# Evrytania/LTE-Cell-Scanner

Measured on AMD Instinct MI355X. Metric: capture-buffers/s (1.92 Msps, 153600-samp) full CellSearch; HBM GB/s vs peak, higher is better.
Workload: dtype i8 x 3 base-256 digits of 24-bit integer templates, i32 accumulate (exact)

## Files before the change

__graft_entry__.py:

```python
from __future__ import annotations

import importlib.util
import os
import subprocess
import sys

ROOT = os.path.dirname(os.path.abspath(__file__))
PKG_DIR = os.path.join(ROOT, "lte-cell-scanner_amd")
CSRC = os.path.join(PKG_DIR, "csrc")
LIB = os.path.join(PKG_DIR, "liblcs_amd.so")
HIP_SOURCES = ["pss_xcorr.hip", "pss_xcorr_i8.hip", "pss_xcorr_f16.hip", "peak_search.hip", "sss_foe.hip", "tfg_mib.hip", "cell_meas.hip", "tfg_wide.hip", "pcfich.hip", "pdcch.hip", "pdsch.hip", "tracker.hip", "channelizer.hip", "channelizer_rate.hip", "lcs_api.hip", "lte_tables.cpp"]
HIPCC_FLAGS = ["--offload-arch=gfx950", "-O3", "-std=c++17", "-ffp-contract=off", "-fPIC", "-shared",
               "-Wall", "-Wno-unused-function"]


_CHAN_DEPS = [os.path.join(CSRC, "channelizer.h"), os.path.join(CSRC, "lcs_internal.h"), os.path.join(ROOT, "include", "lcs.h")]
HOST_TWINS = [
    ("vit_host.cpp", "libvit_host.so", [os.path.join(CSRC, "lte_device.h")], []),
    ("cut_host.cpp", "libcut_host.so", [os.path.join(CSRC, "lte_device.h")], []),
    ("probe_host.cpp", "libprobe_host.so", [os.path.join(CSRC, "lte_device.h")], ["-pthread"]),
    ("pss_ref_host.cpp", "libpss_ref_host.so", [os.path.join(CSRC, "pss_ref.h"), os.path.join(CSRC, "lcs_internal.h"), os.path.join(CSRC, "xcorr_route.h")], []),
    ("chan_rate_host.cpp", "libchan_rate_host.so", _CHAN_DEPS, []),
    ("chan_u8_host.cpp", "libchan_u8_host.so", _CHAN_DEPS, []),
    ("chan_args_host.cpp", "libchan_args_host.so", _CHAN_DEPS, []),
    ("chan_stream_host.cpp", "libchan_stream_host.so", _CHAN_DEPS, []),
    ("chan_stream_u8_host.cpp", "libchan_stream_u8_host.so", _CHAN_DEPS, []),
    ("screen_bound_host.cpp", "libscreen_bound_host.so", [os.path.join(CSRC, "screen_bound.h")], []),
    ("xc_route_host.cpp", "libxc_route_host.so", [os.path.join(CSRC, "xcorr_route.h")], []),
    ("foe_coarse_host.cpp", "libfoe_coarse_host.so", [os.path.join(CSRC, "foe_coarse.h"), os.path.join(CSRC, "lte_device.h")], []),
    ("tdd_config_host.cpp", "libtdd_config_host.so", [os.path.join(CSRC, "tdd_config.h"), os.path.join(CSRC, "lte_device.h")], []),
    ("cell_meas_host.cpp", "libcell_meas_host.so", [os.path.join(CSRC, "cell_meas.h"), os.path.join(CSRC, "tdd_config.h"), os.path.join(CSRC, "lte_device.h")], []),
    ("meas_wide_host.cpp", "libmeas_wide_host.so", [os.path.join(CSRC, "cell_meas_wide.h"), os.path.join(CSRC, "cell_meas.h"), os.path.join(CSRC, "tdd_config.h"), os.path.join(CSRC, "lte_device.h")], []),
    ("pcfich_host.cpp", "libpcfich_host.so", [os.path.join(CSRC, "pcfich.h"), os.path.join(CSRC, "cell_meas.h"), os.path.join(CSRC, "tdd_config.h"), os.path.join(CSRC, "lte_device.h"), os.path.join(ROOT, "include", "lcs.h")], []),
    ("pdcch_host.cpp", "libpdcch_host.so", [os.path.join(CSRC, "pdcch.h"), os.path.join(CSRC, "pcfich.h"), os.path.join(CSRC, "cell_meas.h"), os.path.join(CSRC, "tdd_config.h"), os.path.join(CSRC, "lte_device.h"), os.path.join(ROOT, "include", "lcs.h")], []),
    ("pdsch_host.cpp", "libpdsch_host.so", [os.path.join(CSRC, "pdsch.h"), os.path.join(CSRC, "pdcch.h"), os.path.join(CSRC, "pcfich.h"), os.path.join(CSRC, "cell_meas.h"), os.path.join(CSRC, "tdd_config.h"), os.path.join(CSRC, "lte_device.h"), os.path.join(ROOT, "include", "lcs.h")], []),
    ("pdsch_comb_host.cpp", "libpdsch_comb_host.so", [os.path.join(ROOT, "tests", "host", "pdsch_host.cpp"), os.path.join(CSRC, "pdsch_comb.h"), os.path.join(CSRC, "pdsch.h"), os.path.join(CSRC, "pdcch.h"), os.path.join(CSRC, "pcfich.h"), os.path.join(CSRC, "cell_meas.h"), os.path.join(CSRC, "tdd_config.h"), os.path.join(CSRC, "lte_device.h"), os.path.join(ROOT, "include", "lcs.h")], []),
    ("pdsch_dvrb_host.cpp", "libpdsch_dvrb_host.so", [os.path.join(ROOT, "tests", "host", "pdsch_host.cpp"), os.path.join(CSRC, "pdsch.h"), os.path.join(CSRC, "pdcch.h"), os.path.join(CSRC, "pcfich.h"), os.path.join(CSRC, "cell_meas.h"), os.path.join(CSRC, "tdd_config.h"), os.path.join(CSRC, "lte_device.h"), os.path.join(ROOT, "include", "lcs.h")], []),
    ("pbch_host.cpp", "libpbch_host.so", [os.path.join(CSRC, "lte_tables.cpp"), os.path.join(CSRC, "lcs_internal.h")], []),
    ("trk_layout_host.cpp", "libtrk_layout_host.so", [os.path.join(CSRC, "trk_layout.h"), os.path.join(ROOT, "include", "lcs.h")], []),
]


def load_package():
    name = "lte_cell_scanner_amd"
    if name in sys.modules:
        return sys.modules[name]
    path = os.path.join(PKG_DIR, "__init__.py")
    spec = importlib.util.spec_from_file_location(name, path, submodule_search_locations=[PKG_DIR])
    mod = importlib.util.module_from_spec(spec)
    sys.modules[name] = mod
    spec.loader.exec_module(mod)
    return mod


def _newer(target, sources):
    if not os.path.exists(target):
        return True
    t = os.path.getmtime(target)
    return any(os.path.getmtime(s) > t for s in sources)


def build(force: bool = False) -> None:
    hipcc = os.environ.get("HIPCC", "/opt/rocm/bin/hipcc")
    srcs = [os.path.join(CSRC, s) for s in HIP_SOURCES if os.path.exists(os.path.join(CSRC, s))]
    deps = srcs + [os.path.join(CSRC, "lcs_internal.h"), os.path.join(CSRC, "lcs_mem.h"), os.path.join(CSRC, "channelizer.h"), os.path.join(CSRC, "lte_device.h"), os.path.join(CSRC, "foe_coarse.h"), os.path.join(CSRC, "tdd_config.h"), os.path.join(CSRC, "cell_meas.h"), os.path.join(CSRC, "cell_meas_wide.h"), os.path.join(CSRC, "pcfich.h"), os.path.join(CSRC, "pdcch.h"), os.path.join(CSRC, "pdsch.h"), os.path.join(CSRC, "pdsch_comb.h"), os.path.join(CSRC, "tfg_layout.h"), os.path.join(CSRC, "trk_layout.h"), os.path.join(CSRC, "pss_ref.h"), os.path.join(CSRC, "xcorr_route.h"), os.path.join(CSRC, "screen_bound.h"), os.path.join(ROOT, "include", "lcs.h")]
    if force or _newer(LIB, deps):
        subprocess.check_call([hipcc] + HIPCC_FLAGS + ["-o", LIB] + srcs)
    mk = os.path.join(ROOT, "host", "Makefile")
    if os.path.exists(mk):
        subprocess.check_call(["make", "-C", os.path.dirname(mk), "-s"] + (["-B"] if force else []))
    subprocess.check_call(["make", "-C", os.path.join(ROOT, "oracle"), "-s"])
    for src, lib, extra_deps, extra_flags in HOST_TWINS:
        src, lib = os.path.join(ROOT, "tests", "host", src), os.path.join(ROOT, "tests", "host", lib)
        if os.path.exists(src) and (force or _newer(lib, [src] + extra_deps)):
            subprocess.check_call([hipcc, "--offload-arch=gfx950", "-O2", "-std=c++17", "-ffp-contract=off", "-fPIC", "-shared"] + extra_flags +
                                  ["-I" + os.path.join(ROOT, "include"), "-o", lib, src])
    pkg = load_package()
    pkg.capi.load()


def smoke() -> None:
    import numpy as np
    sys.path.insert(0, os.path.join(ROOT, "oracle"))
    import oracle as O
    pkg = load_package()
    g = np.load(os.path.join(ROOT, "tests", "golden", "capbuf_0000.npz"))
    iq = g["iq_u8"].astype(np.float64)
    cap = ((iq[0::2] - 127.0) / 128.0) + 1j * ((iq[1::2] - 127.0) / 128.0)
    fc = float(g["fc"][0])
    f = np.array([30e3, 35e3, 40e3])
    with pkg.Searcher(0) as s:
        r = s.xcorr_pss(cap, f, 2, fc, fc, 1.92e6, want_incoherent=False)
        Z = pkg.z_th1(r["sp_incoherent"], r["n_comb_xc"])
        peaks = s.peak_search(r["pow"], r["frq"], Z, f, fc, fc, r["single"], 2)
        r32 = s.xcorr_pss(0.5 * cap, f, 2, fc, fc, 1.92e6, want_incoherent=False)
        assert s.last_xcorr_info()[0].startswith("k_xcorr_mfma_blk"), s.last_xcorr_info()
    O.set_threads(min(8, os.cpu_count() or 1))
    ro = O.xcorr_pss(cap, f, 2, fc, fc, 1.92e6)
    assert np.array_equal(r32["frq"], ro["frq"]), "fp32 kernel: collapsed frequency indices differ from the oracle"
    assert np.allclose(4.0 * r32["pow"], ro["pow"], rtol=1e-5, atol=0)
    rel = np.abs(r["single"] - ro["single"]).max() / ro["single"].max()
    assert np.array_equal(r["frq"], ro["frq"]), "int8 kernel: collapsed frequency indices differ from the oracle"
    assert np.allclose(r["pow"], ro["pow"], rtol=1e-5, atol=0), "collapsed powers differ from the oracle"
    po = O.peak_search(ro["pow"], ro["frq"], O.z_th1(ro["sp_incoherent"], ro["n_comb_xc"]), f, fc, fc, ro["single"], 2)
    assert [(p.n_id_2, p.ind, p.freq) for p in peaks] == [(p.n_id_2, p.ind, p.freq) for p in po]
    import torch
    d = torch.from_numpy(np.ascontiguousarray(g["iq_u8"])).to("cuda:0")
    with pkg.Searcher(0) as s:
        cells = s.search_batch(d.data_ptr(), pkg.FMT_IQ_U8, 1, cap.size, f, fc, fc, 1.92e6, pkg.STAGE_FULL)[0]
    co, _ = O.search_capbuf(cap, f, fc, fc, 1.92e6)
# ... 20 lines not shown
```

lte-cell-scanner_amd/csrc/lcs_internal.h:

```cpp
#pragma once
#include <hip/hip_runtime.h>
#include <stdint.h>
#include <cstddef>
#include <string>
#include <type_traits>
#include <vector>
#include "../../include/lcs.h"
#include "lcs_mem.h"
#include "trk_layout.h"
#include "xcorr_route.h"

#define FS_LTE 30720000.0
#define LCS_NW_MAX 16
#define LCS_NF_LIMIT 1024
#define LCS_TAIL_PRIO() __builtin_amdgcn_s_setprio(3)
#define LCS_TG 16
#define LCS_LAG_TILE 64
#define LCS_PS 336
#define LCS_MAXP LCS_MAX_PEAKS
#define LCS_FRQ_TIE_EPS 4e-6f
#define LCS_I8_KB 5
#define LCS_I8_IMG 17024
#define LCS_I8_LAGS 512
#define LCS_I8_TILES ((LCS_N_IDX + LCS_I8_LAGS - 1) / LCS_I8_LAGS)
// ... 97 lines not shown
  int peak;
};

enum class FrqRepair {
  all,
  peaks_only,
  none_keep_2nd
};
struct Launch {
  int n_buf = 0;
  uint32_t n_cap = 0;
  XcGeom geo{};
  const SlotParams *params = nullptr;
  const double *fset = nullptr;
  XcKernel xc = XcKernel::fp32;
  CapSrc src{};
  FrqRepair repair = FrqRepair::all;
  bool screen = false;
  bool single_stream = false;
  bool needed_rows_only = false;
  int grid_items = 64;
  int round_cells = 0;
  int tfoec_parts = 4;
  const int16_t *tracked = nullptr;
  const int *n_tracked = nullptr;
  int duplex = LCS_DUPLEX_FDD;
  int foe_unwrap = 0;
  int tdd_config = 0;
  int cell_meas = 0;
};
struct BatchRecord {
  Launch l;
  int stage_mask = 0;
  int fmt = 0;
  int cell_rounds = 0;
  bool list_ops_counted = false;
};

struct StreamHost {
  SlotParams p;
  int n_tracked;
  int pad_;
  int16_t tracked[504];
  double f;
  lcs_cell res[LCS_MAXP];
  int n_peaks;
  int n_work[4];
};

#define LCS_STREAM_IN_BYTES (offsetof(StreamHost, f) + sizeof(double))

struct TrkStreamCell {
  std::vector<double> fo, ft, late;
  double bpo_before_tail = 0;
  long long tail_start = 0;
  long long n_seen = 0;
  long long next_raw[4] = {1, 1, 1, 1};
  long long ce_upto[4] = {0, 0, 0, 0};
  long long mib_next = 0;
  int cp_type = 0, n_id_1 = -1, n_id_2 = -1, n_ports = 0;
};
struct TrkStream {
  std::vector<TrkStreamCell> cells;
  DevBuf<double2> d_tail[3], d_spare[3];
};
struct TrkCutCap { size_t n_cells = 0, n = 0; };
template <int FIRST, int N, class Cap> struct TrkPart {
  DevBuf<char> buf[N];
  Cap cap;
  template <class T> T *at(const TrkLay &l, int a) const { return l.at<T>(buf[TRK_ROWS[a].buf - FIRST].get(), a); }
  int regrow(lcs_ctx *c, const TrkLay &l, const Cap &want);
  int reserve(lcs_ctx *c, TrkShape s) { return trk_fits(cap, s) ? LCS_OK : regrow(c, trk_layout(trk_grow(cap, s)), trk_grow(cap, s)); }
};

struct I8Set {
  DevBuf<uint16_t> cap8;
  DevBuf<uint16_t> cap8s;
  DevBuf<uint32_t> brow8;
  DevBuf<double> tq;
  DevBuf<float> tsc;
  DevBuf<int> scr_state;
  DevBuf<int> scr_tile;
  DevBuf<unsigned> scr_items;
  DevBuf<float> scr_zmin;
  bool ready = false;
};
struct F16Set {
  DevBuf<uint32_t> cap16h, cap16l;
  DevBuf<uint32_t> brow16;
  DevBuf<int> texp16;
  DevBuf<float> tsc16;
  DevBuf<unsigned> xmax16;
  DevBuf<unsigned> xpart16;
  bool ready = false;
};
struct XcBufs {
  I8Set i8;
  F16Set f16;
  DevBuf<float> btab;
};

struct lcs_ctx;
template <class Rec> struct SideTable {
  explicit SideTable(int sentinel_word) : sentinel(sentinel_word) {}
  DevBuf<Rec> tab;
  bool made = false;
  const int sentinel;
  Rec *get() const { return tab.get(); }
  int begin(lcs_ctx *c, int n_buf, bool on);
  int read_last(lcs_ctx *c, int n_buf, const Rec &none, int32_t Rec::*key, Rec *out, int max_cells_per_buf);
};

struct lcs_ctx_queues {
  int device = 0;
  hipStream_t stream = nullptr;
  hipStream_t stream_xc = nullptr;
  hipEvent_t ev_pre = nullptr, ev_post = nullptr;
  hipEvent_t ev_xc0 = nullptr, ev_xc1 = nullptr;
  hipEvent_t ev_stage[2] = {nullptr, nullptr};
  hipEvent_t ev_chan_slot[2] = {nullptr, nullptr};
  hipEvent_t ev_chan0 = nullptr, ev_chan1 = nullptr;
  ~lcs_ctx_queues();
};

struct lcs_ctx : lcs_ctx_queues {
  ~lcs_ctx();
  std::string err;

  int cap_slots = 0;
  uint32_t cap_n_cap = 0;
  int cap_n_f = 0;
  int cap_G = 0;
  bool cap_debug = false;

  DevBuf<float2> cap32;
  XcBufs xcb;
  DevBuf<double2> cap64;
  DevBuf<SlotParams> params_ws;
  DevBuf<double> fset_ws;
  DevBuf<float2> tmpl;
  DevBuf<int> start, smin, kp2;
  DevBuf<float> single, incoh, sref;
  DevBuf<double> pow_, work, spinc, zth, sp;
  DevBuf<int> frq;
  DevBuf<unsigned> fix_list;
  DevBuf<int> n_fix;
  DevBuf<float> second32;
  DevBuf<double> fset_g;
  DevBuf<lcs_cell> peaks;
  DevBuf<int> npeaks;
  DevBuf<float2> xc;
  DevBuf<WorkItem> pk_items;
  DevBuf<int> n_pk;
  DevBuf<double> sss_ws;
  DevBuf<WorkItem> work_items;
  DevBuf<int> n_work;
  DevBuf<double2> tfg;
  DevBuf<double2> tfg_comp;
  DevBuf<double2> ce;
  DevBuf<char> tfg_desc;
  DevBuf<double> tfg_ts;
  DevBuf<double> tfg_ts_comp;
  DevBuf<double> cell_scratch;
  DevBuf<lcs_cell> cells_out;
  DevBuf<double2> d_pss_td;
  DevBuf<double2> d_pss_fd;
  DevBuf<int8_t> d_sss_fd;
// ... 267 lines not shown
```

lte-cell-scanner_amd/csrc/pss_xcorr.hip:

```cpp
#include "lcs_internal.h"
#include "lte_device.h"
#include "pss_ref.h"
#include <algorithm>

typedef float f32x4 __attribute__((ext_vector_type(4)));

#define NW LCS_NW_MAX
#define NFM geo.n_f
#define GM geo.G

__global__ void k_ingest(const void *__restrict__ src, int fmt, uint32_t n_cap, float2 *__restrict__ cap32,
                         const double2 *__restrict__ cap64) {
  LCS_TAIL_PRIO();
  const int slot = blockIdx.y;
  const size_t base = (size_t)slot * n_cap;
  for (uint32_t i = blockIdx.x * blockDim.x + threadIdx.x; i < n_cap; i += gridDim.x * blockDim.x) {
    if (fmt == LCS_FMT_C64) {
      cap32[base + i] = ((const float2 *)src)[base + i];
    } else {
      const double2 v = cap64[base + i];
      cap32[base + i] = make_float2((float)v.x, (float)v.y);
    }
  }
}
// ... 333 lines not shown
  const int slot = blockIdx.y, i0 = blockIdx.x * SPI_TILE, tid = threadIdx.x, lane = tid & 63, wv = tid >> 6;
  const uint16_t *cap = cap8 + (size_t)slot * lcs_cap8_stride(n_cap);
  double acc[4] = {0, 0, 0, 0};
  for (int m = 0; m < a.n_comb_sp; ++m) {
    const uint32_t base = (uint32_t)m * 9600u + i0;
    int v[SPI_PER], run = 0;
#pragma unroll
    for (int j = 0; j < SPI_PER; ++j) {
      const int k = tid * SPI_PER + j;
      int pw = 0;
      if (k < SPI_N && base + k < n_cap) {
        const uint32_t s = cap[base + k];
        const int re = (int)(int8_t)(s & 255u), im = (int)(int8_t)(s >> 8);
        pw = re * re + im * im;
      }
      run += pw;
      v[j] = run;
    }
    int incl = run;
#pragma unroll
    for (int off = 1; off < 64; off <<= 1) { const int up = __shfl_up(incl, off); if (lane >= off) incl += up; }
    __syncthreads();
    if (lane == 63) wsum[wv] = incl;
    __syncthreads();
    int before = incl - run;
    for (int q = 0; q < wv; ++q) before += wsum[q];
    if (tid == 0) C[0] = 0;
#pragma unroll
    for (int j = 0; j < SPI_PER; ++j) { const int k = tid * SPI_PER + j; if (k < SPI_N) C[k + 1] = before + v[j]; }
    __syncthreads();
#pragma unroll
    for (int r = 0; r < 4; ++r) {
      const int i = tid + 256 * r;
      if (i < SPI_TILE) acc[r] += ((double)(C[i + 274] - C[i]) / 16384.0) / 274;
    }
  }
#pragma unroll
  for (int r = 0; r < 4; ++r) {
    const int i = i0 + tid + 256 * r;
    if (tid + 256 * r < SPI_TILE && i < 9600) {
      const double vv = acc[r] / a.n_comb_sp;
      const int o = (i + 137) % 9600;
      spinc[(size_t)slot * 9600 + o] = vv;
      zth[(size_t)slot * 9600 + o] = lcs_z_th1(a, vv);
    }
  }
}

struct CollapseBest { float v; int foi; float s; };
__device__ __forceinline__ void collapse_step(CollapseBest &b, float xe, int foi) {
  const bool tk = xe > b.v;
  b.s = __builtin_amdgcn_fmed3f(xe, b.v, b.s);
  b.v = tk ? xe : b.v;
  b.foi = tk ? foi : b.foi;
}
__device__ __forceinline__ void collapse_merge(CollapseBest &b, int lane_xor) {
  const float ov = __shfl_xor(b.v, lane_xor);
  const float os = __shfl_xor(b.s, lane_xor);
  const int of = __shfl_xor(b.foi, lane_xor);
  const bool tk = ov > b.v || (ov == b.v && of < b.foi);
  b.s = fmaxf(fminf(b.v, ov), fmaxf(b.s, os));
  b.v = tk ? ov : b.v;
  b.foi = tk ? of : b.foi;
}
__device__ __forceinline__ void collapse_flag(const CollapseBest &r, unsigned pos, unsigned *__restrict__ fix_list, int *__restrict__ n_fix,
                                              const double *__restrict__ zth) {
  if (!fix_list) return;
  if (r.v > 0.f && r.s >= r.v * (1.0f - LCS_FRQ_TIE_EPS)) {
    if (zth && (double)r.v < 0.999 * zth[(pos / (3 * LCS_N_IDX)) * LCS_N_IDX + pos % LCS_N_IDX]) return;
    fix_list[atomicAdd(n_fix, 1)] = pos;
  }
}
typedef const __attribute__((address_space(1))) char *collapse_gptr;
typedef float collapse_f4 __attribute__((ext_vector_type(4)));
__device__ __forceinline__ float4 collapse_row(collapse_gptr base, unsigned byte_off) {
  const collapse_f4 r = *reinterpret_cast<const __attribute__((address_space(1))) collapse_f4 *>(base + byte_off);
  return make_float4(r.x, r.y, r.z, r.w);
}
template <int DS, bool INCOH, bool LIST = false>
__global__ __launch_bounds__(256) void k_collapse(const float *__restrict__ sg, float *__restrict__ incoh,
                                                   double *__restrict__ pow_, float *__restrict__ pow32,
                                                   int *__restrict__ frq, unsigned *__restrict__ fix_list, int *__restrict__ n_fix,
                                                   const double *__restrict__ zth, float *__restrict__ second32, XcGeom geo, int n_buf,
                                                   const int *__restrict__ tile_flag = nullptr, const float *__restrict__ zmin = nullptr) {
  LCS_TAIL_PRIO();
  constexpr int CT = 64;
  static_assert(LCS_N_IDX % CT == 0 && LCS_TG == 16, "k_collapse tiles 9600 positions x 16 columns");
  constexpr int NT = LCS_N_IDX / CT;
  constexpr int NA = DS > 0 ? DS : 1;
  const int tid = threadIdx.x, q = tid & 3;
  const int ds = (DS >= 0) ? DS : min(geo.ds, 8);
  const float dsn = (float)(2 * geo.ds + 1);
  for (int vb = blockIdx.x; vb < NT * n_buf; vb += gridDim.x) {
    const int slot = vb / NT;
    const int idx = (vb % NT) * CT + (tid >> 2);
    bool mine = true;
    if (LIST) {
      static_assert(LCS_I8_LAGS % CT == 0, "a workgroup's positions lie in one lag tile");
      const int *tf = tile_flag + slot * LCS_I8_TILES;
      const int t0 = (vb % NT) * CT / LCS_I8_LAGS;
      if (!tf[t0]) continue;
      const int lo = idx - ds < 0 ? idx - ds + LCS_N_IDX : idx - ds, hi = idx + ds >= LCS_N_IDX ? idx + ds - LCS_N_IDX : idx + ds;
      mine = tf[lo / LCS_I8_LAGS] && tf[hi / LCS_I8_LAGS];
    }
    const unsigned o0 = ((unsigned)idx * 4u + q) * 16u;
    unsigned om[NA], op[NA];
#pragma unroll
    for (int d = 1; d <= DS; ++d) {
      om[d - 1] = ((unsigned)((idx - d < 0) ? idx - d + LCS_N_IDX : idx - d) * 4u + q) * 16u;
      op[d - 1] = ((unsigned)((idx + d >= LCS_N_IDX) ? idx + d - LCS_N_IDX : idx + d) * 4u + q) * 16u;
    }
    CollapseBest b0 = {-INFINITY, 0, -INFINITY}, b1 = {-INFINITY, 0, -INFINITY}, b2 = {-INFINITY, 0, -INFINITY};
#pragma unroll 1
    for (int g = 0; g < geo.G; ++g) {
      const uintptr_t gb = reinterpret_cast<uintptr_t>(sg + (((size_t)slot * geo.G + g) * LCS_N_IDX) * LCS_TG);
      const unsigned gb_hi = (unsigned)__builtin_amdgcn_readfirstlane((int)(gb >> 32)), gb_lo = (unsigned)__builtin_amdgcn_readfirstlane((int)(unsigned)gb);
      const collapse_gptr rows = reinterpret_cast<collapse_gptr>(((uintptr_t)gb_hi << 32) | (uintptr_t)gb_lo);
      float4 v = collapse_row(rows, o0);
      if (DS >= 0) {
        float4 a[NA], b[NA];
#pragma unroll
        for (int d = 1; d <= DS; ++d) { a[d - 1] = collapse_row(rows, om[d - 1]); b[d - 1] = collapse_row(rows, op[d - 1]); }
#pragma unroll
        for (int d = 1; d <= DS; ++d) {
          v.x = v.x + (a[d - 1].x + b[d - 1].x); v.y = v.y + (a[d - 1].y + b[d - 1].y);
          v.z = v.z + (a[d - 1].z + b[d - 1].z); v.w = v.w + (a[d - 1].w + b[d - 1].w);
        }
      } else {
        for (int d = 1; d <= ds; ++d) {
          const int im = (idx - d < 0) ? idx - d + LCS_N_IDX : idx - d, ip = (idx + d >= LCS_N_IDX) ? idx + d - LCS_N_IDX : idx + d;
          const float4 a = collapse_row(rows, ((unsigned)im * 4u + q) * 16u), b = collapse_row(rows, ((unsigned)ip * 4u + q) * 16u);
          v.x = v.x + (a.x + b.x); v.y = v.y + (a.y + b.y); v.z = v.z + (a.z + b.z); v.w = v.w + (a.w + b.w);
        }
      }
      const int cq = g * geo.cpg + 4 * q;
      const int f0 = cq / 3, t0 = cq - 3 * f0;
      float vv[4] = {__fdiv_rn(v.x, dsn), __fdiv_rn(v.y, dsn), __fdiv_rn(v.z, dsn), __fdiv_rn(v.w, dsn)};
      asm volatile("" : "+v"(vv[0]), "+v"(vv[1]), "+v"(vv[2]), "+v"(vv[3]));
#pragma unroll
      for (int j = 0; j < 4; ++j) {
        const int tj = t0 + j;
        const int t = (tj >= 3) ? tj - 3 : tj, foi = f0 + (tj >= 3 ? 1 : 0);
        const bool valid = (4 * q + j < geo.cpg) && (cq + j < geo.n_tmpl);
        const float x = vv[j];
        if (INCOH) { if (valid) incoh[((((size_t)slot * 3 + t) * LCS_N_IDX) + idx) * geo.n_f + foi] = x; }
        collapse_step(b0, (valid && t == 0) ? x : -INFINITY, foi);
        collapse_step(b1, (valid && t == 1) ? x : -INFINITY, foi);
        collapse_step(b2, (valid && t == 2) ? x : -INFINITY, foi);
      }
    }
    collapse_merge(b0, 1); collapse_merge(b0, 2);
    collapse_merge(b1, 1); collapse_merge(b1, 2);
    collapse_merge(b2, 1); collapse_merge(b2, 2);
    if (q < 3 && mine) {
      const CollapseBest r = (q == 0) ? b0 : (q == 1 ? b1 : b2);
      const size_t o = ((size_t)slot * 3 + q) * LCS_N_IDX + idx;
      pow_[o] = (double)r.v;
      pow32[o] = r.v;
      frq[o] = r.foi;
      if (second32) second32[o] = r.s;
      if (LIST) { if (r.v < 0.999f * zmin[slot]) continue; }
      collapse_flag(r, (unsigned)o, fix_list, n_fix, zth);
    }
  }
}

template <int CTRL>
__device__ __forceinline__ float collapse_dpp(float x) {
  return __int_as_float(__builtin_amdgcn_update_dpp(0, __float_as_int(x), CTRL, 0xf, 0xf, true));
}
__device__ __forceinline__ float collapse_arm2(float me) {
  float v = me + (collapse_dpp<0x111>(me) + collapse_dpp<0x101>(me));
  return v + (collapse_dpp<0x112>(me) + collapse_dpp<0x102>(me));
}
__device__ __forceinline__ float collapse_div5(float x) {
  const float q = x * 0.2f;
  return fmaf(fmaf(-5.0f, q, x), 0.2f, q);
}
typedef unsigned int collapse_u4 __attribute__((ext_vector_type(4)));
#define COLLAPSE_OUT 12
#define COLLAPSE_GB 3
__global__ __launch_bounds__(256) __attribute__((amdgpu_num_vgpr(28))) void k_collapse_arm2(const float *__restrict__ sg, double *__restrict__ pow_, float *__restrict__ pow32,
                                                        int *__restrict__ frq, unsigned *__restrict__ fix_list, int *__restrict__ n_fix,
                                                        const double *__restrict__ zth, float *__restrict__ second32, XcGeom geo, int n_buf) {
  LCS_TAIL_PRIO();
  constexpr int CT = 4 * COLLAPSE_OUT;
  static_assert(LCS_N_IDX % CT == 0 && LCS_TG == 16, "k_collapse_arm2 tiles 9600 positions x 16 columns");
  constexpr int NT = LCS_N_IDX / CT;
  const int tid = threadIdx.x, lane = tid & 63, p = lane & 15, q = lane >> 4, wv = tid >> 6;
  for (int vb = blockIdx.x; vb < NT * n_buf; vb += gridDim.x) {
    const int slot = vb / NT;
    const int idx = (vb % NT) * CT + wv * COLLAPSE_OUT + p - 2;
    const int ridx = idx < 0 ? idx + LCS_N_IDX : (idx >= LCS_N_IDX ? idx - LCS_N_IDX : idx);
    const unsigned off = ((unsigned)ridx * 4u + q) * 16u;
    CollapseBest acc[3] = {{-INFINITY, 0, -INFINITY}, {-INFINITY, 0, -INFINITY}, {-INFINITY, 0, -INFINITY}};
    const __amdgpu_buffer_rsrc_t rsrc = __builtin_amdgcn_make_buffer_rsrc(
        const_cast<float *>(sg + ((size_t)slot * geo.G * LCS_N_IDX) * LCS_TG), 0, geo.G * (int)(LCS_N_IDX * LCS_TG * sizeof(float)), 0x00020000);
    constexpr int GROUP_BYTES = (int)(LCS_N_IDX * LCS_TG * sizeof(float));
    for (int g6 = 0; g6 < geo.G; g6 += COLLAPSE_GB) {
      collapse_u4 me[COLLAPSE_GB];
      if (g6 + COLLAPSE_GB <= geo.G) {
#pragma unroll
        for (int r = 0; r < COLLAPSE_GB; ++r) me[r] = __builtin_amdgcn_raw_buffer_load_b128(rsrc, (int)off, (g6 + r) * GROUP_BYTES, 0);
      } else {
#pragma unroll
        for (int r = 0; r < COLLAPSE_GB; ++r) {
          me[r] = __builtin_amdgcn_raw_buffer_load_b128(rsrc, (int)off, (g6 + r) * GROUP_BYTES, 0);
        }
      }
      const int cb = g6 * 16 + 4 * q;
#pragma unroll
      for (int r = 0; r < COLLAPSE_GB; ++r) {
        const float mv[4] = {__uint_as_float(me[r].x), __uint_as_float(me[r].y), __uint_as_float(me[r].z), __uint_as_float(me[r].w)};
#pragma unroll
        for (int j = 0; j < 4; ++j) {
          const float x = collapse_div5(collapse_arm2(mv[j]));
          const int col = cb + (16 * r + j);
          collapse_step(acc[(r + j) % 3], (col < geo.n_tmpl) ? x : -INFINITY, col);
        }
      }
    }
    const int k0 = (3 - q) % 3, k1 = (4 - q) % 3, k2 = (5 - q) % 3;
    CollapseBest o0 = (k0 == 0) ? acc[0] : (k0 == 1 ? acc[1] : acc[2]);
    CollapseBest o1 = (k1 == 0) ? acc[0] : (k1 == 1 ? acc[1] : acc[2]);
    CollapseBest o2 = (k2 == 0) ? acc[0] : (k2 == 1 ? acc[1] : acc[2]);
    collapse_merge(o0, 16); collapse_merge(o0, 32);
    collapse_merge(o1, 16); collapse_merge(o1, 32);
    collapse_merge(o2, 16); collapse_merge(o2, 32);
    if (q < 3 && p >= 2 && p < 2 + COLLAPSE_OUT) {
      const CollapseBest rb = (q == 0) ? o0 : (q == 1 ? o1 : o2);
      const float rv = rb.v;
      const int rf = rb.foi / 3;
      int oi = idx;
      asm volatile("" : "+v"(oi));
      const size_t o = ((size_t)slot * 3 + q) * LCS_N_IDX + oi;
      pow_[o] = (double)rv;
      pow32[o] = rv;
      frq[o] = rf;
      if (second32) second32[o] = rb.s;
      collapse_flag(rb, (unsigned)o, fix_list, n_fix, zth);
    }
  }
}

// ... 326 lines not shown

static int xc_hand_over(lcs_ctx *c, hipStream_t sxc) {
  HIPCHK(c, hipEventRecord(c->ev_pre, c->stream));
  HIPCHK(c, hipStreamWaitEvent(sxc, c->ev_pre, 0));
  std::lock_guard<std::mutex> lk(g_xc_mutex);
  hipEvent_t &ev = g_xc_done[c->device & 63];
  if (!ev) HIPCHK(c, hipEventCreateWithFlags(&ev, hipEventDisableTiming | LCS_EVENT_NOFENCE));
  else HIPCHK(c, hipStreamWaitEvent(sxc, ev, 0));
  return LCS_OK;
}
static int xc_hand_back(lcs_ctx *c, hipStream_t sxc) {
  {
    std::lock_guard<std::mutex> lk(g_xc_mutex);
    HIPCHK(c, hipEventRecord(g_xc_done[c->device & 63], sxc));
  }
  HIPCHK(c, hipEventRecord(c->ev_post, sxc));
  HIPCHK(c, hipStreamWaitEvent(c->stream, c->ev_post, 0));
  return LCS_OK;
}

static void xc_signal_power(lcs_ctx *c, const Launch &L) {
  const XcGeom &geo = L.geo;
  const int n_buf = L.n_buf;
  const SpArgs a = make_sp_args(geo);
  if (L.src.c8) {
    hipLaunchKernelGGL(k_sp_i8, dim3(LCS_N_IDX / SPI_TILE, n_buf), dim3(256), 0, c->stream, c->xcb.i8.cap8, geo.n_cap, c->spinc, c->zth, a);
  } else {
    hipLaunchKernelGGL(k_sp_sums, dim3(((LCS_N_IDX + SP_TILE - 1) / SP_TILE) * a.n_comb_sp * n_buf), dim3(64), 0,
                       c->stream, L.src, c->sp, geo.n_cap, a.n_comb_sp, n_buf);
    hipLaunchKernelGGL(k_sp_fold, dim3((n_buf * LCS_N_IDX + 255) / 256), dim3(256), 0, c->stream, c->sp, c->spinc, c->zth, a, n_buf);
  }
}

static int xc_correlate(lcs_ctx *c, hipStream_t sxc, const Launch &L, bool time_it) {
  const int n_buf = L.n_buf;
  const int n8 = (n_buf >= 8 && L.xc != XcKernel::single_exact) ? (n_buf & ~7) : 0;
  if (time_it) HIPCHK(c, hipEventRecord(c->ev_xc0, sxc));
  int launches = 0;
  c->last_xc_ops = 0;
  for (int part = 0; part < 2; ++part) {
    const int s0 = part ? n8 : 0, ns = part ? n_buf - n8 : n8;
    if (ns <= 0) continue;
    if (int rc = xc_launch_part(c, sxc, L, s0, ns, part ? 0 : 1)) return rc;
    ++launches;
  }
  if (time_it) { HIPCHK(c, hipEventRecord(c->ev_xc1, sxc)); c->last_xc_launches = launches; }
  return LCS_OK;
}

static void xc_collapse(lcs_ctx *c, const Launch &L, bool want_incoh) {
  const XcGeom &geo = L.geo;
  const int n_buf = L.n_buf;
  const dim3 grid((LCS_N_IDX / 64) * n_buf), block(256);
  float *incoh = want_incoh ? c->incoh : nullptr;
  float *pow32 = reinterpret_cast<float *>(c->work.get());
  const double *zf = L.repair == FrqRepair::peaks_only ? c->zth : nullptr;
  float *s2 = L.repair == FrqRepair::none_keep_2nd ? c->second32 : nullptr;
  unsigned *fix_list = L.screen ? nullptr : c->fix_list.get();
  if (geo.ds == 2 && !incoh && geo.cpg == LCS_TG)
    hipLaunchKernelGGL(k_collapse_arm2, dim3((LCS_N_IDX / (4 * COLLAPSE_OUT)) * n_buf), block, 0, c->stream, c->single, c->pow_, pow32, c->frq, fix_list, c->n_fix, zf, s2, geo, n_buf);
  else if (geo.ds == 2 && !incoh) hipLaunchKernelGGL((k_collapse<2, false>), grid, block, 0, c->stream, c->single, incoh, c->pow_, pow32, c->frq, fix_list, c->n_fix, zf, s2, geo, n_buf);
  else if (!incoh) hipLaunchKernelGGL((k_collapse<-1, false>), grid, block, 0, c->stream, c->single, incoh, c->pow_, pow32, c->frq, fix_list, c->n_fix, zf, s2, geo, n_buf);
  else hipLaunchKernelGGL((k_collapse<-1, true>), grid, block, 0, c->stream, c->single, incoh, c->pow_, pow32, c->frq, fix_list, c->n_fix, zf, s2, geo, n_buf);
}

static void xc_tie_repair(lcs_ctx *c, const Launch &L) {
  const XcGeom &geo = L.geo;
  if (L.repair == FrqRepair::none_keep_2nd || geo.n_f <= 1) return;
  const int ng = std::min(512, std::max(64, 8 * L.n_buf));
  float *pow32 = reinterpret_cast<float *>(c->work.get());
  lcs_by_cap_kind(L.src, [&](auto kind) {
    hipLaunchKernelGGL((k_frq_repair<decltype(kind)::value, false>), dim3(ng), dim3(REPAIR_THREADS), 0, c->stream, c->single, c->fix_list, c->n_fix, L.src,
                       L.params, L.fset, c->d_pss_td, c->start, c->pow_, pow32, c->frq, nullptr, nullptr, c->zth, c->n_fix + 1, geo);
  });
}

static int xc_screen_refine(lcs_ctx *c, const Launch &L) {
  const XcGeom &geo = L.geo;
  if (int rc = lcs_launch_screen_refine(c, L)) return rc;
  float *pow32 = reinterpret_cast<float *>(c->work.get());
  const dim3 grid((LCS_N_IDX / 64) * L.n_buf), block(256);
  if (geo.ds == 2)
    hipLaunchKernelGGL((k_collapse<2, false, true>), grid, block, 0, c->stream, c->single, nullptr, c->pow_, pow32, c->frq, c->fix_list, c->n_fix, nullptr, nullptr, geo, L.n_buf,
                       c->xcb.i8.scr_tile, c->xcb.i8.scr_zmin);
  else
    hipLaunchKernelGGL((k_collapse<-1, false, true>), grid, block, 0, c->stream, c->single, nullptr, c->pow_, pow32, c->frq, c->fix_list, c->n_fix, nullptr, nullptr, geo, L.n_buf,
                       c->xcb.i8.scr_tile, c->xcb.i8.scr_zmin);
  return LCS_OK;
}

int lcs_launch_xcorr(lcs_ctx *c, const Launch &L, bool want_incoh, bool time_it) {
  hipStream_t sxc = L.single_stream ? c->stream : c->stream_xc;
  int rc;
  if (L.screen && (L.xc != XcKernel::i8 || want_incoh || L.repair != FrqRepair::all)) { c->err = "the screen serves int8 batches"; return LCS_ERR_BAD_ARG; }
  c->screen_pending = false;
  if ((rc = xc_tables_and_operands(c, L))) return rc;
  if (!L.single_stream && (rc = xc_hand_over(c, sxc))) return rc;
  xc_signal_power(c, L);
  if ((rc = xc_correlate(c, sxc, L, time_it))) return rc;
  if (!L.single_stream && (rc = xc_hand_back(c, sxc))) return rc;
  xc_collapse(c, L, want_incoh);
  if (L.screen && (rc = xc_screen_refine(c, L))) return rc;
  xc_tie_repair(c, L);
  HIPCHK(c, hipGetLastError());
  c->screen_pending = L.screen;
  return LCS_OK;
}

int lcs_launch_xcorr_complete(lcs_ctx *c, const Launch &L_batch) {
  if (!c->screen_pending) return LCS_OK;
  Launch L = L_batch;
  L.screen = false;
  hipStream_t sxc = L.single_stream ? c->stream : c->stream_xc;
  const double ops = c->last_xc_ops;
  int rc;
  HIPCHK(c, hipMemsetAsync(c->n_fix, 0, 2 * sizeof(int), c->stream));
  if (!L.single_stream && (rc = xc_hand_over(c, sxc))) return rc;
  if ((rc = xc_correlate(c, sxc, L, false))) return rc;
  if (!L.single_stream && (rc = xc_hand_back(c, sxc))) return rc;
  c->last_xc_ops = ops;
  xc_collapse(c, L, false);
  xc_tie_repair(c, L);
  HIPCHK(c, hipGetLastError());
  c->screen_pending = false;
  return LCS_OK;
}

int lcs_launch_foe_contend(lcs_ctx *c, const Launch &L, const double *fset_g, const long long *d_words, long long *d_words2) {
  const XcGeom &geo = L.geo;
  const CapSrc &cs = L.src;
  HIPCHK(c, hipMemsetAsync(c->n_fix, 0, 2 * sizeof(int), c->stream));
  float *pow32 = reinterpret_cast<float *>(c->work.get());
  hipLaunchKernelGGL(k_foe_flag, dim3((3 * LCS_N_IDX + 255) / 256), dim3(256), 0, c->stream, d_words, pow32, c->second32, d_words2, c->fix_list, c->n_fix, geo);
  lcs_by_cap_kind(cs, [&](auto kind) {
    hipLaunchKernelGGL((k_frq_repair<decltype(kind)::value, true>), dim3(512), dim3(REPAIR_THREADS), 0, c->stream, c->single, c->fix_list, c->n_fix, cs,
                       L.params, fset_g, c->d_pss_td, c->start, c->pow_, pow32, c->frq, d_words, d_words2, c->zth, c->n_fix + 1, geo);
  });
  HIPCHK(c, hipGetLastError());
  return LCS_OK;
}
int lcs_launch_foe_resolve(lcs_ctx *c, long long *d_words, const long long *d_words2) {
  hipLaunchKernelGGL(k_foe_resolve, dim3((3 * LCS_N_IDX + 255) / 256), dim3(256), 0, c->stream, d_words, d_words2);
  HIPCHK(c, hipGetLastError());
  return LCS_OK;
}

int lcs_launch_single_layout(lcs_ctx *c, const Launch &L, int slot, float *ref_layout, int to_ref) {
  const XcGeom &geo = L.geo;
  float *sg = c->single + (size_t)slot * geo.G * LCS_N_IDX * LCS_TG;
  hipLaunchKernelGGL(k_single_to_ref, dim3(256, 1), dim3(256), 0, c->stream, sg, ref_layout, geo, to_ref);
  HIPCHK(c, hipGetLastError());
  return LCS_OK;
}

int lcs_launch_xc_debug(lcs_ctx *c, const Launch &L) {
  const XcGeom &geo = L.geo;
  hipLaunchKernelGGL(k_xc_debug, dim3(64, geo.n_f, 3), dim3(256), 0, c->stream, c->cap64, L.params, L.fset,
                     c->d_pss_td, c->xc, geo);
  HIPCHK(c, hipGetLastError());
  return LCS_OK;
}
```

lte-cell-scanner_amd/csrc/pss_xcorr_i8.hip:

```cpp
#include "lcs_internal.h"
#include "screen_bound.h"
#include <algorithm>

typedef float f32x4 __attribute__((ext_vector_type(4)));
typedef int i32x4 __attribute__((ext_vector_type(4)));

#define NW LCS_NW_MAX
#define NFM geo.n_f
#define GM geo.G

#ifndef I8_MT
#define I8_MT 8
#endif
#define I8_LAGS (4 * I8_MT * 16)
#define I8_TILES ((LCS_N_IDX + I8_LAGS - 1) / I8_LAGS)
#define I8_NKB LCS_I8_KB
#define I8_PCPY 144
static_assert(I8_PCPY >= (15 + 24) / 2 + 8 * (2 * (I8_NKB - 1) + I8_MT - 1) + 4 && I8_PCPY % 32 == 16 && I8_PCPY % 4 == 0, "sample staging");
#define I8_QMAX 8300000.0

#define I8R_OFF LCS_I8_OFF
#define I8R_ROW 88
#define I8R_RLEN 88
#define I8R_BLK 1412
// ... 177 lines not shown
        const int d1 = (e + 1) / I8_NKB, j1 = (e + 1) % I8_NKB;
        const int kb1 = (d1 == 1) ? I8_NKB - 1 - j1 : j1;
#pragma unroll
        for (int op = 0; op < 2; ++op) I8_RD_B(2 - d1, kb1, op, Bq[(e + 1) & 1][op]);
        if (kb1 > kb) { I8_RD_A(2 * kb1 + I8_MT - 2); I8_RD_A(2 * kb1 + I8_MT - 1); }
        else if (kb1 < kb) { I8_RD_A(2 * kb1); I8_RD_A(2 * kb1 + 1); }
      }
      __builtin_amdgcn_sched_barrier(0);
#pragma unroll
      for (int mt = 1; mt < I8_MT; ++mt) I8_PF_MFMA(mt);
      if (ND == 3 && d == 1) {
#pragma unroll
        for (int mt = j; mt < I8_MT; mt += I8_NKB)
#pragma unroll
          for (int r = 0; r < 4; ++r) { fR[mt][r] = (float)tR[mt][r]; fI[mt][r] = (float)tI[mt][r]; }
      }
      __builtin_amdgcn_sched_barrier(0);
    }
#undef I8_PF_MFMA
#pragma unroll
    for (int mt = 0; mt < I8_MT; ++mt)
#pragma unroll
      for (int r = 0; r < 4; ++r) {
        const float xr = ND == 3 ? fmaf(fR[mt][r], 65536.f, (float)aR[mt][r]) : (float)aR[mt][r];
        const float xi = ND == 3 ? fmaf(fI[mt][r], 65536.f, (float)aI[mt][r]) : (float)aI[mt][r];
        P[mt][r] = fmaf(xi, xi, fmaf(xr, xr, P[mt][r]));
      }
  };
  dma(0, ldsA0);
  __syncthreads();
  if (widx0 >= LCS_N_IDX) return;
  for (int w = 0; w < geo.n_comb; w += 2) {
    window(w, ldsA0, ldsA1);
    if (w + 1 < geo.n_comb) window(w + 1, ldsA1, ldsA0);
  }
#undef I8_RD_A
#undef I8_DELAY_AND_PREFETCH
#undef I8_RD_B
  const float ncomb = (float)geo.n_comb;
  const float col_sc = sc[(size_t)slot * GM * LCS_TG + g * LCS_TG + (lane & 15)];
  const float my_sc = ND == 3 ? col_sc : col_sc * 256.f;
  float *o = sg + (((size_t)slot * geo.G + g) * LCS_N_IDX) * LCS_TG + (lane & 15);
#pragma unroll
  for (int mt = 0; mt < I8_MT; ++mt)
#pragma unroll
    for (int r = 0; r < 4; ++r) {
      const int idx = widx0 + mt * 16 + 4 * (lane >> 4) + r;
      if (idx < LCS_N_IDX) o[(size_t)idx * LCS_TG] = __fdiv_rn(P[mt][r] * (my_sc * my_sc), ncomb);
    }
}

static_assert(I8_TILES <= 32, "a work item keeps its lag tile in five bits");
#define I8_ITEM_SLOTS 65536
#define I8_ITEM_GROUPS 2048
__host__ __device__ static inline unsigned i8_item(int slot, int g, int tile) { return ((unsigned)slot << 16) | ((unsigned)g << 5) | (unsigned)tile; }

template <int ND, bool LIST>
__global__ __launch_bounds__(256, 2) void k_xcorr_i8x3(const uint16_t *__restrict__ cap8, const uint16_t *__restrict__ cap8s,
                                                          const int *__restrict__ smin, const int *__restrict__ start,
                                                          const uint32_t *__restrict__ brow,
                                                          const float *__restrict__ sc, float *__restrict__ sg, XcGeom geo,
                                                          int slot0, int n_slots, int xcd_map,
                                                          const unsigned *__restrict__ items, const int *__restrict__ n_items) {
  if (LIST) {
    const int n = *n_items;
    for (int i = blockIdx.x; i < n; i += gridDim.x) {
      if (i != (int)blockIdx.x) __syncthreads();
      const unsigned it = (unsigned)__builtin_amdgcn_readfirstlane((int)items[i]);
      int tid = threadIdx.x;
      asm volatile("" : "+v"(tid));
      i8_tile<ND>(cap8, cap8s, smin, start, brow, sc, sg, geo, (int)(it >> 16), (int)((it >> 5) & (I8_ITEM_GROUPS - 1)), (int)(it & 31u) * I8_LAGS, tid);
    }
  } else {
    const int per_slot = I8_TILES * geo.G;
    int q, sidx;
    if (xcd_map) { sidx = blockIdx.x & 7; q = blockIdx.x >> 3; sidx += 8 * (q / per_slot); q = q % per_slot; }
    else { sidx = blockIdx.x / per_slot; q = blockIdx.x % per_slot; }
    if (sidx >= n_slots) return;
    i8_tile<ND>(cap8, cap8s, smin, start, brow, sc, sg, geo, slot0 + sidx, q / I8_TILES, (q % I8_TILES) * I8_LAGS, threadIdx.x);
  }
}

__global__ __launch_bounds__(256) void k_screen_flag(const float *__restrict__ pow32, const double *__restrict__ zth, const float *__restrict__ sc,
                                                     XcGeom geo, float *__restrict__ zmin, int *__restrict__ state, int *__restrict__ tile_flag,
                                                     unsigned *__restrict__ items) {
  LCS_TAIL_PRIO();
  const int slot = blockIdx.x, tid = threadIdx.x;
  __shared__ double s_z[4];
  __shared__ float s_sc[4];
  __shared__ int s_bad[4];
  __shared__ int s_flag[I8_TILES];
  const double *z = zth + (size_t)slot * LCS_N_IDX;
  double zm = INFINITY;
  int bad = 0;
  for (int i = tid; i < LCS_N_IDX; i += 256) { const double v = z[i]; bad |= !(v > 0.0); zm = fmin(zm, v); }
  float sm = 0.f;
  for (int i = tid; i < geo.G * LCS_TG; i += 256) sm = fmaxf(sm, sc[(size_t)slot * GM * LCS_TG + i]);
  for (int o = 32; o; o >>= 1) { zm = fmin(zm, __shfl_xor(zm, o)); sm = fmaxf(sm, __shfl_xor(sm, o)); }
  bad = __any(bad);
  if ((tid & 63) == 0) { s_z[tid >> 6] = zm; s_sc[tid >> 6] = sm; s_bad[tid >> 6] = bad; }
  if (tid < I8_TILES) s_flag[tid] = 0;
  __syncthreads();
  zm = fmin(fmin(s_z[0], s_z[1]), fmin(s_z[2], s_z[3]));
  sm = fmaxf(fmaxf(s_sc[0], s_sc[1]), fmaxf(s_sc[2], s_sc[3]));
  bad = s_bad[0] | s_bad[1] | s_bad[2] | s_bad[3];
  const double T = bad ? -1.0 : lcs_screen_threshold(geo.n_comb, geo.ds, (double)sm, zm);
  const bool all = !(T > 0.0);
  const float *pw = pow32 + (size_t)slot * 3 * LCS_N_IDX;
  if (all) { if (tid < I8_TILES) s_flag[tid] = 1; }
  else
    for (int e = tid; e < 3 * LCS_N_IDX; e += 256) {
      if ((double)pw[e] < T) continue;
      const int idx = e % LCS_N_IDX;
      const int lo = idx - geo.ds < 0 ? idx - geo.ds + LCS_N_IDX : idx - geo.ds, hi = idx + geo.ds >= LCS_N_IDX ? idx + geo.ds - LCS_N_IDX : idx + geo.ds;
      s_flag[idx / I8_LAGS] = 1; s_flag[lo / I8_LAGS] = 1; s_flag[hi / I8_LAGS] = 1;
    }
  __syncthreads();
  if (tid < I8_TILES) {
    const int f = s_flag[tid];
    tile_flag[slot * I8_TILES + tid] = f;
    if (f) {
      const int at = atomicAdd(state, geo.G);
      for (int g = 0; g < geo.G; ++g) items[at + g] = i8_item(slot, g, tid);
      atomicAdd(state + 1, 1);
      if (tid == I8_TILES - 1) atomicAdd(state + 3, 1);
    }
  }
  if (tid == 0) {
    float zf = (float)zm;
    if ((double)zf > zm) zf = __uint_as_float(__float_as_uint(zf) - 1u);
    zmin[slot] = all ? 0.f : zf;
    if (all) atomicAdd(state + 2, 1);
  }
}

int lcs_launch_fill_brow_i8(lcs_ctx *c, const Launch &L) {
  const int n_buf = L.n_buf;
  const XcGeom &geo = L.geo;
  hipLaunchKernelGGL(k_i8_scales, dim3(n_buf), dim3(256), 0, c->stream, c->tmpl, c->xcb.i8.tq, c->xcb.i8.tsc, geo);
  hipLaunchKernelGGL(k_fill_brow_i8, dim3((LCS_TG * 2 * I8R_RLEN + 255) / 256, geo.G, n_buf), dim3(256), 0, c->stream, c->tmpl, c->xcb.i8.tq, c->xcb.i8.brow8, geo);
  HIPCHK(c, hipGetLastError());
  return LCS_OK;
}
int lcs_launch_xcorr_i8(lcs_ctx *c, hipStream_t sxc, const Launch &L, int slot0, int n_slots, int xcd_map) {
  const XcGeom &geo = L.geo;
  const unsigned grid = (unsigned)(I8_TILES * geo.G * n_slots);
  const I8Set &s = c->xcb.i8;
  if (L.screen)
    hipLaunchKernelGGL((k_xcorr_i8x3<2, false>), dim3(grid), dim3(256), 0, sxc, s.cap8, s.cap8s, c->smin, c->start, s.brow8, s.tsc, c->single, geo, slot0, n_slots, xcd_map,
                       nullptr, nullptr);
  else
    hipLaunchKernelGGL((k_xcorr_i8x3<3, false>), dim3(grid), dim3(256), 0, sxc, s.cap8, s.cap8s, c->smin, c->start, s.brow8, s.tsc, c->single, geo, slot0, n_slots, xcd_map,
                       nullptr, nullptr);
  HIPCHK(c, hipGetLastError());
  const double waves = (double)n_slots * geo.G * ((LCS_N_IDX + I8_MT * 16 - 1) / (I8_MT * 16));
  c->last_xc_ops += waves * geo.n_comb * ((L.screen ? 2.0 : 3.0) * I8_NKB * I8_MT * 2) * (2.0 * 16 * 16 * 64);
  c->last_xc_kernel = "k_xcorr_i8x3";
  return LCS_OK;
}
double lcs_i8_list_ops(const XcGeom &geo, int tiles, int last_tiles) {
  static_assert(LCS_I8_LAGS == I8_LAGS && LCS_I8_TILES == I8_TILES, "lcs_internal.h names the kernel's tiling");
  const double waves = (double)geo.G * (4.0 * tiles - (4 - (LCS_N_IDX - (I8_TILES - 1) * I8_LAGS + I8_MT * 16 - 1) / (I8_MT * 16)) * (double)last_tiles);
  return waves * geo.n_comb * (3.0 * I8_NKB * I8_MT * 2) * (2.0 * 16 * 16 * 64);
}
int lcs_launch_screen_refine(lcs_ctx *c, const Launch &L) {
  const XcGeom &geo = L.geo;
  I8Set &s = c->xcb.i8;
  const size_t S = (size_t)c->cap_slots;
  if (L.n_buf > I8_ITEM_SLOTS || geo.G > I8_ITEM_GROUPS) { c->err = "batch too large for the screen's work items"; return LCS_ERR_BAD_ARG; }
  if (s.scr_tile.capacity() < S * I8_TILES || s.scr_items.capacity() < S * I8_TILES * (size_t)c->cap_G) {
    if (c->st_open) { c->err = "the screen's buffers cannot be allocated while a stream is open: lcs_stream_close first"; return LCS_ERR_BAD_ARG; }
    HIPCHK(c, hipStreamSynchronize(c->stream));
    int rc;
    if ((rc = s.scr_state.alloc(c, 4)) || (rc = s.scr_tile.alloc(c, S * I8_TILES)) || (rc = s.scr_items.alloc(c, S * I8_TILES * (size_t)c->cap_G)) ||
        (rc = s.scr_zmin.alloc(c, S)))
      return rc;
  }
  HIPCHK(c, hipMemsetAsync(s.scr_state, 0, 4 * sizeof(int), c->stream));
  hipLaunchKernelGGL(k_screen_flag, dim3(L.n_buf), dim3(256), 0, c->stream, reinterpret_cast<const float *>(c->work.get()), c->zth, s.tsc, geo, s.scr_zmin, s.scr_state,
                     s.scr_tile, s.scr_items);
  int cus = 256;
  (void)hipDeviceGetAttribute(&cus, hipDeviceAttributeMultiprocessorCount, c->device);
  const unsigned grid = (unsigned)std::min<long long>(2LL * cus, (long long)L.n_buf * I8_TILES * geo.G);
  hipLaunchKernelGGL((k_xcorr_i8x3<3, true>), dim3(grid), dim3(256), 0, c->stream, s.cap8, s.cap8s, c->smin, c->start, s.brow8, s.tsc, c->single, geo, 0, L.n_buf, 0,
                     s.scr_items, s.scr_state);
  HIPCHK(c, hipGetLastError());
  return LCS_OK;
}
```

lte-cell-scanner_amd/csrc/screen_bound.h:

```cpp
#pragma once
#include <cmath>

#if defined(__HIP__) || defined(__host__)
#define LCS_SCREEN_HD __host__ __device__
#else
#define LCS_SCREEN_HD
#endif

LCS_SCREEN_HD static inline double lcs_screen_err(double sc) { return (1.4142135623730951 * 128.0 * 274.0 * 128.0) * sc; }
LCS_SCREEN_HD static inline double lcs_screen_bound(double e, double v) { return 2.0 * e * sqrt(v) + e * e; }
LCS_SCREEN_HD static inline double lcs_screen_slack(int n_comb, int ds) { return ldexp(4.0 * (double)(n_comb + 2 * ds + 1) + 16.0, -23) + 4e-7; }
LCS_SCREEN_HD static inline double lcs_screen_threshold(int n_comb, int ds, double sc, double Z) {
  const double e = lcs_screen_err(sc);
  if (!(Z > 0.0) || !(sc > 0.0) || !(Z < INFINITY) || !(e < INFINITY)) return -1.0;
  if (!(Z > e * e)) return -1.0;
  const double T = (Z - lcs_screen_bound(e, Z)) * (1.0 - lcs_screen_slack(n_comb, ds));
  return T > 0.0 ? T : -1.0;
}
```

Measured before the change: 63110.

## Tighten screen threshold using per-slot lower bound of surviving peaks

```diff
diff --git a/__graft_entry__.py b/__graft_entry__.py
--- a/__graft_entry__.py
+++ b/__graft_entry__.py
@@ -26,6 +26,7 @@
     ("chan_stream_host.cpp", "libchan_stream_host.so", _CHAN_DEPS, []),
     ("chan_stream_u8_host.cpp", "libchan_stream_u8_host.so", _CHAN_DEPS, []),
     ("screen_bound_host.cpp", "libscreen_bound_host.so", [os.path.join(CSRC, "screen_bound.h")], []),
+    ("screen_theta_host.cpp", "libscreen_theta_host.so", [os.path.join(CSRC, "screen_bound.h")], []),
     ("xc_route_host.cpp", "libxc_route_host.so", [os.path.join(CSRC, "xcorr_route.h")], []),
     ("foe_coarse_host.cpp", "libfoe_coarse_host.so", [os.path.join(CSRC, "foe_coarse.h"), os.path.join(CSRC, "lte_device.h")], []),
     ("tdd_config_host.cpp", "libtdd_config_host.so", [os.path.join(CSRC, "tdd_config.h"), os.path.join(CSRC, "lte_device.h")], []),
diff --git a/lte-cell-scanner_amd/csrc/lcs_internal.h b/lte-cell-scanner_amd/csrc/lcs_internal.h
--- a/lte-cell-scanner_amd/csrc/lcs_internal.h
+++ b/lte-cell-scanner_amd/csrc/lcs_internal.h
@@ -203,7 +203,7 @@
   DevBuf<int> scr_state;
   DevBuf<int> scr_tile;
   DevBuf<unsigned> scr_items;
-  DevBuf<float> scr_zmin;
+  DevBuf<float> scr_theta;
   bool ready = false;
 };
 struct F16Set {
diff --git a/lte-cell-scanner_amd/csrc/pss_xcorr.hip b/lte-cell-scanner_amd/csrc/pss_xcorr.hip
--- a/lte-cell-scanner_amd/csrc/pss_xcorr.hip
+++ b/lte-cell-scanner_amd/csrc/pss_xcorr.hip
@@ -439,7 +439,7 @@
                                                    double *__restrict__ pow_, float *__restrict__ pow32,
                                                    int *__restrict__ frq, unsigned *__restrict__ fix_list, int *__restrict__ n_fix,
                                                    const double *__restrict__ zth, float *__restrict__ second32, XcGeom geo, int n_buf,
-                                                   const int *__restrict__ tile_flag = nullptr, const float *__restrict__ zmin = nullptr) {
+                                                   const int *__restrict__ tile_flag = nullptr, const float *__restrict__ theta = nullptr) {
   LCS_TAIL_PRIO();
   constexpr int CT = 64;
   static_assert(LCS_N_IDX % CT == 0 && LCS_TG == 16, "k_collapse tiles 9600 positions x 16 columns");
@@ -516,7 +516,7 @@
       pow32[o] = r.v;
       frq[o] = r.foi;
       if (second32) second32[o] = r.s;
-      if (LIST) { if (r.v < 0.999f * zmin[slot]) continue; }
+      if (LIST) { if (r.v < 0.999f * theta[slot]) continue; }
       collapse_flag(r, (unsigned)o, fix_list, n_fix, zth);
     }
   }
@@ -1009,10 +1009,10 @@
   const dim3 grid((LCS_N_IDX / 64) * L.n_buf), block(256);
   if (geo.ds == 2)
     hipLaunchKernelGGL((k_collapse<2, false, true>), grid, block, 0, c->stream, c->single, nullptr, c->pow_, pow32, c->frq, c->fix_list, c->n_fix, nullptr, nullptr, geo, L.n_buf,
-                       c->xcb.i8.scr_tile, c->xcb.i8.scr_zmin);
+                       c->xcb.i8.scr_tile, c->xcb.i8.scr_theta);
   else
     hipLaunchKernelGGL((k_collapse<-1, false, true>), grid, block, 0, c->stream, c->single, nullptr, c->pow_, pow32, c->frq, c->fix_list, c->n_fix, nullptr, nullptr, geo, L.n_buf,
-                       c->xcb.i8.scr_tile, c->xcb.i8.scr_zmin);
+                       c->xcb.i8.scr_tile, c->xcb.i8.scr_theta);
   return LCS_OK;
 }
 
diff --git a/lte-cell-scanner_amd/csrc/pss_xcorr_i8.hip b/lte-cell-scanner_amd/csrc/pss_xcorr_i8.hip
--- a/lte-cell-scanner_amd/csrc/pss_xcorr_i8.hip
+++ b/lte-cell-scanner_amd/csrc/pss_xcorr_i8.hip
@@ -283,18 +283,23 @@
 }
 
 __global__ __launch_bounds__(256) void k_screen_flag(const float *__restrict__ pow32, const double *__restrict__ zth, const float *__restrict__ sc,
-                                                     XcGeom geo, float *__restrict__ zmin, int *__restrict__ state, int *__restrict__ tile_flag,
+                                                     XcGeom geo, float *__restrict__ theta_out, int *__restrict__ state, int *__restrict__ tile_flag,
                                                      unsigned *__restrict__ items) {
   LCS_TAIL_PRIO();
   const int slot = blockIdx.x, tid = threadIdx.x;
-  __shared__ double s_z[4];
+  __shared__ double s_z[4], s_l[4];
   __shared__ float s_sc[4];
-  __shared__ int s_bad[4];
+  __shared__ int s_bad[4], s_badv[4];
   __shared__ int s_flag[I8_TILES];
   const double *z = zth + (size_t)slot * LCS_N_IDX;
   double zm = INFINITY;
   int bad = 0;
-  for (int i = tid; i < LCS_N_IDX; i += 256) { const double v = z[i]; bad |= !(v > 0.0); zm = fmin(zm, v); }
+  static_assert(LCS_N_IDX % 4 == 0, "a float4 of pow32 lies within one PSS; a double2 of zth within the buffer");
+  for (int i = tid; i < LCS_N_IDX / 2; i += 256) {
+    const double2 v = reinterpret_cast<const double2 *>(z)[i];
+    bad |= !(v.x > 0.0 && v.x < INFINITY) | !(v.y > 0.0 && v.y < INFINITY);
+    zm = fmin(zm, fmin(v.x, v.y));
+  }
   float sm = 0.f;
   for (int i = tid; i < geo.G * LCS_TG; i += 256) sm = fmaxf(sm, sc[(size_t)slot * GM * LCS_TG + i]);
   for (int o = 32; o; o >>= 1) { zm = fmin(zm, __shfl_xor(zm, o)); sm = fmaxf(sm, __shfl_xor(sm, o)); }
@@ -305,16 +310,47 @@
   zm = fmin(fmin(s_z[0], s_z[1]), fmin(s_z[2], s_z[3]));
   sm = fmaxf(fmaxf(s_sc[0], s_sc[1]), fmaxf(s_sc[2], s_sc[3]));
   bad = s_bad[0] | s_bad[1] | s_bad[2] | s_bad[3];
-  const double T = bad ? -1.0 : lcs_screen_threshold(geo.n_comb, geo.ds, (double)sm, zm);
-  const bool all = !(T > 0.0);
+  const double Tmin = bad ? -1.0 : lcs_screen_threshold(geo.n_comb, geo.ds, (double)sm, zm);
   const float *pw = pow32 + (size_t)slot * 3 * LCS_N_IDX;
-  if (all) { if (tid < I8_TILES) s_flag[tid] = 1; }
-  else
-    for (int e = tid; e < 3 * LCS_N_IDX; e += 256) {
-      if ((double)pw[e] < T) continue;
-      const int idx = e % LCS_N_IDX;
-      const int lo = idx - geo.ds < 0 ? idx - geo.ds + LCS_N_IDX : idx - geo.ds, hi = idx + geo.ds >= LCS_N_IDX ? idx + geo.ds - LCS_N_IDX : idx + geo.ds;
-      s_flag[idx / I8_LAGS] = 1; s_flag[lo / I8_LAGS] = 1; s_flag[hi / I8_LAGS] = 1;
+  int mode = LCS_SCREEN_ALL;
+  float theta = 0.f;
+  double T = -1.0;
+  if (Tmin > 0.0) {
+    const float pre = (float)(0.999 * Tmin);
+    double lm = INFINITY;
+    int badv = 0;
+    for (int q = tid; q < 3 * LCS_N_IDX / 4; q += 256) {
+      const float4 v4 = reinterpret_cast<const float4 *>(pw)[q];
+      const float vv[4] = {v4.x, v4.y, v4.z, v4.w};
+#pragma unroll
+      for (int j = 0; j < 4; ++j) {
+        const float v = vv[j];
+        badv |= !(v > 0.f && v < INFINITY);
+        if (v < pre) continue;
+        if (!lcs_screen_in_s(geo.n_comb, geo.ds, (double)sm, z[(4 * q + j) % LCS_N_IDX], (double)v)) continue;
+        lm = fmin(lm, lcs_screen_lower(geo.n_comb, geo.ds, (double)sm, (double)v));
+      }
+    }
+    for (int o = 32; o; o >>= 1) lm = fmin(lm, __shfl_xor(lm, o));
+    badv = __any(badv);
+    if ((tid & 63) == 0) { s_l[tid >> 6] = lm; s_badv[tid >> 6] = badv; }
+    __syncthreads();
+    lm = fmin(fmin(s_l[0], s_l[1]), fmin(s_l[2], s_l[3]));
+    badv = s_badv[0] | s_badv[1] | s_badv[2] | s_badv[3];
+    if (!badv) mode = lcs_screen_decide(geo.n_comb, geo.ds, (double)sm, lm, &theta, &T);
+  }
+  if (mode == LCS_SCREEN_ALL) { if (tid < I8_TILES) s_flag[tid] = 1; }
+  else if (mode == LCS_SCREEN_BY_T)
+    for (int q = tid; q < 3 * LCS_N_IDX / 4; q += 256) {
+      const float4 v4 = reinterpret_cast<const float4 *>(pw)[q];
+      const float vv[4] = {v4.x, v4.y, v4.z, v4.w};
+#pragma unroll
+      for (int j = 0; j < 4; ++j) {
+        if (!lcs_screen_hot(T, (double)vv[j])) continue;
+        const int idx = (4 * q + j) % LCS_N_IDX;
+        const int lo = idx - geo.ds < 0 ? idx - geo.ds + LCS_N_IDX : idx - geo.ds, hi = idx + geo.ds >= LCS_N_IDX ? idx + geo.ds - LCS_N_IDX : idx + geo.ds;
+        s_flag[idx / I8_LAGS] = 1; s_flag[lo / I8_LAGS] = 1; s_flag[hi / I8_LAGS] = 1;
+      }
     }
   __syncthreads();
   if (tid < I8_TILES) {
@@ -328,10 +364,8 @@
     }
   }
   if (tid == 0) {
-    float zf = (float)zm;
-    if ((double)zf > zm) zf = __uint_as_float(__float_as_uint(zf) - 1u);
-    zmin[slot] = all ? 0.f : zf;
-    if (all) atomicAdd(state + 2, 1);
+    theta_out[slot] = theta;
+    if (mode == LCS_SCREEN_ALL) atomicAdd(state + 2, 1);
   }
 }
 
@@ -374,11 +408,11 @@
     HIPCHK(c, hipStreamSynchronize(c->stream));
     int rc;
     if ((rc = s.scr_state.alloc(c, 4)) || (rc = s.scr_tile.alloc(c, S * I8_TILES)) || (rc = s.scr_items.alloc(c, S * I8_TILES * (size_t)c->cap_G)) ||
-        (rc = s.scr_zmin.alloc(c, S)))
+        (rc = s.scr_theta.alloc(c, S)))
       return rc;
   }
   HIPCHK(c, hipMemsetAsync(s.scr_state, 0, 4 * sizeof(int), c->stream));
-  hipLaunchKernelGGL(k_screen_flag, dim3(L.n_buf), dim3(256), 0, c->stream, reinterpret_cast<const float *>(c->work.get()), c->zth, s.tsc, geo, s.scr_zmin, s.scr_state,
+  hipLaunchKernelGGL(k_screen_flag, dim3(L.n_buf), dim3(256), 0, c->stream, reinterpret_cast<const float *>(c->work.get()), c->zth, s.tsc, geo, s.scr_theta, s.scr_state,
                      s.scr_tile, s.scr_items);
   int cus = 256;
   (void)hipDeviceGetAttribute(&cus, hipDeviceAttributeMultiprocessorCount, c->device);
diff --git a/lte-cell-scanner_amd/csrc/screen_bound.h b/lte-cell-scanner_amd/csrc/screen_bound.h
--- a/lte-cell-scanner_amd/csrc/screen_bound.h
+++ b/lte-cell-scanner_amd/csrc/screen_bound.h
@@ -17,3 +17,29 @@
   const double T = (Z - lcs_screen_bound(e, Z)) * (1.0 - lcs_screen_slack(n_comb, ds));
   return T > 0.0 ? T : -1.0;
 }
+
+LCS_SCREEN_HD static inline double lcs_screen_lower(int n_comb, int ds, double sc, double vs) {
+  const double e = lcs_screen_err(sc), k = 1.0 - lcs_screen_slack(n_comb, ds);
+  const double r = sqrt(vs * k) - e;
+  return r > 0.0 ? r * r * k : 0.0;
+}
+LCS_SCREEN_HD static inline bool lcs_screen_in_s(int n_comb, int ds, double sc, double z, double vs) {
+  return !(vs < lcs_screen_threshold(n_comb, ds, sc, z));
+}
+#define LCS_SCREEN_NONE 0
+#define LCS_SCREEN_BY_T 1
+#define LCS_SCREEN_ALL 2
+LCS_SCREEN_HD static inline int lcs_screen_decide(int n_comb, int ds, double sc, double lmin, float *theta, double *T) {
+  *theta = 0.f;
+  *T = -1.0;
+  if (lmin == INFINITY) return LCS_SCREEN_NONE;
+  if (!(lmin > 0.0) || !(lmin < 3.0e38)) return LCS_SCREEN_ALL;
+  float tf = (float)lmin;
+  if ((double)tf > lmin) tf = nextafterf(tf, 0.f);
+  if (!(tf > 0.f)) return LCS_SCREEN_ALL;
+  *T = lcs_screen_threshold(n_comb, ds, sc, (double)tf);
+  if (!(*T > 0.0)) return LCS_SCREEN_ALL;
+  *theta = tf;
+  return LCS_SCREEN_BY_T;
+}
+LCS_SCREEN_HD static inline bool lcs_screen_hot(double T, double vs) { return !(vs < T); }
```

After: 65980, median of 6. +4.6%, better.
